# zrudnick/bramble

Measured on AMD Instinct MI355X. Metric: projected alignments/sec vs GENCODE-scale annotation, higher is better.
Workload: dtype u32

## Files before the change

bramble_amd/csrc/abi.cpp:

```cpp
#include <hip/hip_runtime.h>

#include <algorithm>
#include <atomic>
#include <cstdio>
#include <cstdlib>
#include <cstring>
#include <functional>
#include <string>
#include <thread>
#include <unordered_map>
#include <vector>

#include "ctx.h"
#include "primary_pick.h"

int check_device(int device) {
  int n = 0;
  hipError_t e = hipGetDeviceCount(&n);
  if (e != hipSuccess || n <= 0 || device >= n) return BR_ERR_NO_DEVICE;
  return BR_OK;
}

template <typename T>
static int upload(void **dst, const std::vector<T> &src, size_t &acc) {
// ... 66 lines not shown
  for (int pad = 0; pad < 4; pad++) ix->tx_ex.push_back(make_uint4(0xffffffffu, 0xffffffffu, 0, 0));
  auto for_each_par = [](size_t n, const std::function<void(size_t)> &fn) {
    unsigned hw = std::thread::hardware_concurrency();
    const size_t nt = std::min<size_t>(n, std::max(1u, std::min(hw ? hw : 1u, 16u)));
    if (nt <= 1) { for (size_t i = 0; i < n; i++) fn(i); return; }
    std::atomic<size_t> next{0};
    auto body = [&]() { for (;;) { const size_t i = next.fetch_add(1); if (i >= n) break; fn(i); } };
    std::vector<std::thread> th;
    for (size_t t = 1; t < nt; t++) th.emplace_back(body);
    body();
    for (auto &x : th) x.join();
  };
  ix->slab_off.assign(slabs.size() + 1, 0);
  {
    uint64_t tot = 0;
    for (size_t k = 0; k < slabs.size(); k++) { tot += slabs[k].size(); if (tot >= 0xfffffff0ull) { delete ix; return BR_ERR_CAPACITY; } ix->slab_off[k + 1] = (uint32_t)tot; }
    ix->s_start.resize((size_t)tot); ix->s_pmax.resize((size_t)tot); ix->s_tid.resize((size_t)tot); ix->s_row.resize((size_t)tot * 2);
  }
  for_each_par(slabs.size(), [&](size_t k) {
    auto &rows = slabs[k];
    std::stable_sort(rows.begin(), rows.end(), [](const Row &a, const Row &b) { return a.start < b.start; });
    uint32_t m = 0;
    size_t at = ix->slab_off[k];
    for (auto &r : rows) {
      m = std::max(m, r.end);
      ix->s_start[at] = r.start; ix->s_pmax[at] = m;
      ix->s_row[2 * at] = make_uint4(r.start, r.end, ix->tx_ex[ix->tx_first[r.tid] + r.gidx + 1].x , r.pos_start);
      const uint32_t n_ex = ix->tx_first[r.tid + 1] - ix->tx_first[r.tid] - 1;
      ix->s_row[2 * at + 1] = make_uint4(r.tid, r.gidx | (n_ex > 256u ? 0x80000000u : 0u), ix->tx_first[r.tid], ix->tx_ex[ix->tx_first[r.tid] + r.gidx + 1].y );
      ix->s_tid[at] = r.tid;
      at++;
    }
  });
  const uint32_t SHIFT = 10;
  std::vector<uint64_t> n_bins(ix->n_refs, 2);
  ix->bin_off.assign((size_t)ix->n_refs + 1, 0);
  {
    uint64_t tot = 0;
    for (uint32_t r = 0; r < ix->n_refs; r++) {
      uint64_t nb = 2;
      for (int sd = 0; sd < 2; sd++) {
        uint32_t sb = ix->slab_off[2 * r + sd], se = ix->slab_off[2 * r + sd + 1];
        if (se > sb) nb = std::max<uint64_t>(nb, ((uint64_t)std::max(ix->s_start[se - 1], ix->s_pmax[se - 1]) >> SHIFT) + 2);
      }
      n_bins[r] = nb;
      tot += nb + 1;
      if (tot >= 0xfffffff0ull) { delete ix; return BR_ERR_CAPACITY; }
      ix->bin_off[r + 1] = (uint32_t)tot;
    }
    ix->t_bin.resize((size_t)tot);
  }
  for_each_par(ix->n_refs, [&](size_t r) {
    const uint64_t nb = n_bins[r];
    const size_t first = ix->bin_off[r];
    for (int sd = 0; sd < 2; sd++) {
      uint32_t sb = ix->slab_off[2 * r + sd], se = ix->slab_off[2 * r + sd + 1];
      uint32_t rh = sb, rl = sb;
      for (uint64_t bk = 0; bk <= nb; bk++) {
        if (bk < nb) {
          uint64_t edge = bk << SHIFT;
          while (rh < se && (uint64_t)ix->s_start[rh] < edge) rh++;
          while (rl < se && (uint64_t)ix->s_pmax[rl] <= edge) rl++;
        } else rh = rl = se;
        uint4 &e = ix->t_bin[first + bk];
        if (sd == 0) { e.x = rl; e.y = rh; } else { e.z = rl; e.w = rh; }
      }
    }
// ... 329 lines not shown
```

bramble_amd/csrc/direct_kernels.inc:

```

#define WAVE_SYNC()                                                \
  do {                                                             \
    __builtin_amdgcn_fence(__ATOMIC_RELEASE, "workgroup");         \
    __builtin_amdgcn_wave_barrier();                               \
    __builtin_amdgcn_fence(__ATOMIC_ACQUIRE, "workgroup");         \
  } while (0)

__global__ void __launch_bounds__(256) k_name_seed(DirectArgs D) {
  const int64_t g = (int64_t)blockIdx.x * blockDim.x + threadIdx.x;
  if (g >= D.n_groups) return;
  const uint32_t a0 = D.group_off[g];
  const uint32_t no = D.name_off[a0];
  Mt64Lazy gen;
  gen.seed(hash_bytes(D.names + no, D.name_off[a0 + 1] - no));
  D.rnd0[g] = gen();
}
__device__ __forceinline__ uint32_t pick_from(uint64_t z0, const uint8_t *name, uint64_t len, uint32_t n) {
  uint64_t hi, lo;
  mul64wide(z0, (uint64_t)n, hi, lo);
  if (lo < (uint64_t)n) {
    const uint64_t thr = (0 - (uint64_t)n) % (uint64_t)n;
    if (lo < thr) return primary_pick(name, len, n);
  }
  return (uint32_t)hi;
// ... 416 lines not shown
    for (int k = 0; k < SCAN5_TOP_ITEMS; k++) { if (i0 + k < n_tiles) ts[i0 + k] = ex; ex += v[k]; }
    carry += tot;
  }
  if (threadIdx.x == 0) total_out[blockIdx.x] = carry;
}
__global__ void __launch_bounds__(256) k_scan5_apply(DirectArgs D, const uint64_t *tile_sums, int64_t n_tiles, const uint64_t *totals) {
  __shared__ uint64_t sh[4];
  const int64_t base = (int64_t)blockIdx.x * SCAN_TILE + (int64_t)threadIdx.x * SCAN_ITEMS;
  Scan5 v[SCAN_ITEMS];
  uint64_t sum[4] = {0, 0, 0, 0};
  scan5_load<false>(D, base, v);
#pragma unroll
  for (int k = 0; k < SCAN_ITEMS; k++)
#pragma unroll
    for (int c = 0; c < 4; c++) sum[c] += v[k].v[c];
  uint64_t ex[4];
#pragma unroll
  for (int c = 0; c < 4; c++) { uint64_t tot; ex[c] = block_excl_scan_256(sum[c], sh, tot) + tile_sums[(int64_t)c * n_tiles + blockIdx.x]; }
  const uint32_t n_simple = (uint32_t)totals[2];
  uint32_t o0[SCAN_ITEMS]; uint64_t o1[SCAN_ITEMS], o3[SCAN_ITEMS];
#pragma unroll
  for (int k = 0; k < SCAN_ITEMS; k++) {
    o0[k] = v[k].v[2] ? (uint32_t)ex[2] : n_simple + (uint32_t)(ex[0] - ex[2]);
    o1[k] = ex[1]; o3[k] = ex[3];
#pragma unroll
    for (int c = 0; c < 4; c++) ex[c] += v[k].v[c];
  }
  store8(D.cls_pos, base, D.n_aln, o0); store8(D.cig_base, base, D.n_aln, o1); store8(D.row_off, base, D.n_aln, o3);
  if (blockIdx.x == gridDim.x - 1 && threadIdx.x == 255) { D.cig_base[D.n_aln] = ex[1]; D.row_off[D.n_aln] = ex[3]; }
}

struct __attribute__((packed, aligned(4))) GD4 { uint32_t a, b, c, d; };
__global__ void __launch_bounds__(256) k_group_desc(DirectArgs D) {
  unsigned long long uniq = 0, dropped = 0;
  for (int64_t g = (int64_t)blockIdx.x * blockDim.x + threadIdx.x; g < D.n_groups; g += (int64_t)gridDim.x * blockDim.x) {
    const uint32_t a0 = D.group_off[g], a1 = D.group_off[g + 1];
    const uint32_t na = a1 - a0;
    uint32_t total = 0, units = 0, any = 0;
    uint32_t r4[4] = {0, 0, 0, 0}, f4[4] = {0, 0, 0, 0};
    int32_t mi4[4] = {-1, -1, -1, -1};
    const bool small = na <= 4u;
    if (small) {
      const GD4 rr = *(const GD4 *)(D.n_rows + a0), mm = *(const GD4 *)(D.n_matches + a0);
      typedef uint32_t u32u1 __attribute__((aligned(1)));
      const uint32_t ff = *(const u32u1 *)(D.pflag + a0);
#pragma unroll
      for (int k = 0; k < 4; k++) mi4[k] = (uint32_t)k < na ? D.mate_idx[a0 + (uint32_t)k] : -1;
      r4[0] = rr.a; r4[1] = rr.b; r4[2] = rr.c; r4[3] = rr.d;
      uint32_t m4[4] = {mm.a, mm.b, mm.c, mm.d};
#pragma unroll
      for (int k = 0; k < 4; k++) {
        f4[k] = (ff >> (8 * k)) & 0xffu;
        if ((uint32_t)k >= na) { r4[k] = 0; m4[k] = 0; f4[k] = 0; }
        total += r4[k]; units += (f4[k] & PF_PAIRED) ? r4[k] / 2 : r4[k]; any |= m4[k];
      }
    } else {
      for (uint32_t i = a0; i < a1; i++) { const uint32_t r = D.n_rows[i]; total += r; units += (D.pflag[i] & PF_PAIRED) ? r / 2 : r; any |= D.n_matches[i]; }
    }
    uniq += total == 1u ? 1 : 0;
    dropped += any ? 0 : 1;
    if (total == 0) continue;
    if (total > RR_HI) D.counters[3] = 1;
    const bool have_prim = D.names != nullptr;
    uint32_t idx = 0;
    if (have_prim && units > 1) {
      uint64_t hi, lo;
// ... 34 lines not shown
        const bool paired = (pf & PF_PAIRED) != 0;
        const uint32_t u = paired ? r / 2 : r;
        uint32_t prim = 0;
        if (have_prim && idx != 0xffffffffu) { if (idx < u) { prim = idx + 1u; idx = 0xffffffffu; } else idx -= u; }
        D.gd[i] = make_uint2(pf | (prim << 8), total);
        D.hi0[i] = run + 1u;
        if (paired) {
          const uint32_t m = (uint32_t)D.mate_idx[i];
          D.gd[m] = make_uint2((uint32_t)D.pflag[m] | (prim << 8), total);
          D.hi0[m] = run + 2u;
        }
        run += r;
      }
    }
  }
  __shared__ unsigned long long sh_c[4][2];
#pragma unroll
  for (int d = 32; d >= 1; d >>= 1) { uniq += __shfl_down(uniq, d, 64); dropped += __shfl_down(dropped, d, 64); }
  if ((threadIdx.x & 63) == 0) { sh_c[threadIdx.x >> 6][0] = uniq; sh_c[threadIdx.x >> 6][1] = dropped; }
  __syncthreads();
  if (threadIdx.x == 0) {
    const unsigned long long u = sh_c[0][0] + sh_c[1][0] + sh_c[2][0] + sh_c[3][0], dr = sh_c[0][1] + sh_c[1][1] + sh_c[2][1] + sh_c[3][1];
    uint64_t *slot = D.counters + GD_SLOT0 + (size_t)(blockIdx.x & (GD_SLOTS - 1)) * GD_SLOT_STRIDE;
    if (u) atomicAdd((unsigned long long *)&slot[0], u);
    if (dr) atomicAdd((unsigned long long *)&slot[1], dr);
  }
}

__global__ void __launch_bounds__(256) k_expand_rows(DirectArgs D) {
  __shared__ uint32_t sh_pre[4][64], sh_v[4][64];
  const int lane = threadIdx.x & 63, wv = threadIdx.x >> 6;
  const int64_t a = (int64_t)blockIdx.x * blockDim.x + threadIdx.x;
  if (D.m_aln_cap && D.tot[0] > D.m_aln_cap) return;
  uint32_t nk = 0, pos = 0, v = 0;
  bool fast = false;
  if (a < D.n_aln) nk = D.n_kept[a];
  if (nk) {
    fast = D.fast_flag[a] >> 31;
    pos = D.cls_pos[a];
    const uint32_t y = D.pflag[a];
    const bool is_mate = (y & PF_MATE) != 0;
    const uint32_t leader = is_mate ? (uint32_t)D.mate_idx[a] : (uint32_t)a;
    D.dpos[a] = make_uint2((uint32_t)D.row_off[leader] + (is_mate ? 1u : 0u), pos);
    v = (y & PF_BIG) ? 0xffffffffu : (uint32_t)a;
  }
  sh_v[wv][lane] = v;
#pragma unroll
  for (int c = 0; c < 2; c++) {
    const uint32_t mine = (nk && fast == (c == 0)) ? nk : 0u;
    const uint64_t have = __ballot(mine != 0u);
    if (!have) continue;
    uint32_t inc = mine;
#pragma unroll
    for (int d = 1; d < 64; d <<= 1) { const uint32_t up = __shfl_up(inc, d); if (lane >= d) inc += up; }
    const uint32_t total = __shfl(inc, 63), first = __shfl(pos, (int)__builtin_ctzll(have));
    __builtin_amdgcn_wave_barrier();
    sh_pre[wv][lane] = inc - mine;
    WAVE_SYNC();
    for (uint32_t e = lane; e < total; e += 64) {
      int l = 0;
#pragma unroll
      for (int st = 32; st; st >>= 1) if (sh_pre[wv][l + st] <= e) l += st;
      D.m_aln[first + e] = sh_v[wv][l];
    }
  }
}
// ... 149 lines not shown
```

bramble_amd/csrc/kernels.h:

```cpp
#pragma once
#include <hip/hip_runtime.h>
#include <stdint.h>

#include "device_types.h"
#include "ksw_types.h"

namespace br {

struct ProjectArgs {
  DevIndex ix;
  DevCfg cfg;
  int64_t n_aln;
  const int32_t *ref_id;
  const uint32_t *cigar_off;
  const uint32_t *cigar;
  const uint2 *seg;
  const AlnMeta *meta;
  const uint4 *head;
  const uint4 *head2;
  const uint32_t *fast_flag;
  const uint32_t *fast_pre;
  uint32_t *n_matches;
  uint4 *ranges;
  uint64_t *mask;
  uint32_t *big_list;
  uint32_t *n_big;
  uint32_t *walk_list;
  uint32_t *n_walk;
  uint32_t *m_aln;
  const uint32_t *match_off;
  const uint64_t *cig_base;
  uint32_t *m_tid, *m_aux;
  uint2 *m_p;
  uint2 *m_x;
  uint4 *m_b;
  uint64_t *m_cigoff;
  uint32_t *cig_arena;
  const uint64_t *tot;
  uint64_t lim_m, lim_c;
  uint64_t cover;
};
__device__ __forceinline__ bool tot_over(const uint64_t *tot, uint64_t lim_m, uint64_t lim_c) { return tot && (tot[0] > lim_m || tot[1] > lim_c); }

struct FaArgs {
  const int32_t *seq_src;
  const uint32_t *seq_off;
  const uint8_t *seqs;
  uint32_t *n_prob;
  uint32_t *seq_bytes;
  const uint32_t *prob_off;
  const uint64_t *seqarena_off;
  KswProb *probs;
  FaSrc *srcs;
  KswRes *results;
  uint8_t *seq_arena;
  uint32_t *clip_ops;
  uint32_t *ideal_cap;
  uint64_t *want_l, *want_r;
};

struct KswArgs {
  int64_t n_prob;
  const KswProb *probs;
  KswRes *results;
  const uint8_t *seq_arena;
  uint32_t *clip_ops;
  uint8_t *scratch;
  size_t scratch_per_wave, pmat_bytes, raw_words;
  int64_t n_waves;
  uint32_t tmax;
  uint64_t *stats;
  uint32_t *raw_out, *raw_n; int32_t *max_out; uint32_t raw_cap;
  const uint32_t *list; const uint32_t *n_list;
};

// ... 258 lines not shown
  int32_t *seq_src;
  uint32_t *seq_len;
  const uint32_t *seq_off;
  uint8_t *seqs;
  const int32_t *mate_ref_id, *mate_start;
};
struct SoaArgs {
  int64_t n;
  const uint64_t *cigar_off64, *name_off64, *seq_off64;
  uint32_t *cigar_off, *name_off, *seq_off;
  const uint8_t *names;
  const uint32_t *cigar;
  uint32_t *isnew;
  uint32_t *maxima;
};
void launch_soa_fields(hipStream_t st, const SoaArgs &S);
void launch_rec_fields(hipStream_t st, const ParseArgs &P);
void launch_group_off(hipStream_t st, const ParseArgs &P);
void launch_rec_copy(hipStream_t st, const ParseArgs &P);
void launch_mates(hipStream_t st, const ParseArgs &P);
void launch_seq_src(hipStream_t st, const ParseArgs &P);
void launch_seq_ascii(hipStream_t st, const ParseArgs &P);
void launch_bam_size(hipStream_t st, const BamArgs &B);
void launch_bam_encode(hipStream_t st, const BamArgs &B, int lanes);

struct SegExtra {
  const uint32_t *group_off; uint32_t *aln_group; int64_t n_groups;
  uint64_t *zero_a; int n_zero_a; uint64_t *zero_b; int n_zero_b;
};
void launch_segment(hipStream_t st, int64_t n_aln, const int32_t *ref_id, const int32_t *ref_start,
                    const uint16_t *flags, const int8_t *xs, const int8_t *ts, const uint32_t *cigar_off,
                    const uint32_t *cigar, const DevCfg &cfg, uint32_t n_refs, uint2 *seg, AlnMeta *meta,
                    uint4 *head, uint4 *head2, uint32_t *fast_flag, const SegExtra *extra = nullptr);
void launch_project(hipStream_t st, const ProjectArgs &A, bool emit, int group_lanes, int n_blocks, int part = 0);
void launch_project_fa(hipStream_t st, const ProjectArgs &A, const FaArgs &F, int mode, int n_blocks);
void launch_fa_fill(hipStream_t st, const ProjectArgs &A, const FaArgs &F, int64_t n_prob);
void launch_ksw(hipStream_t st, const KswArgs &K, int n_blocks);
void launch_ksw_bin(hipStream_t st, const KswFastArgs &A);
void launch_ksw_dp(hipStream_t st, const KswFastArgs &A, int bin);
void launch_ksw_trace(hipStream_t st, const KswFastArgs &A, int bin);
uint32_t ksw_dp_resident_groups(int bin, int n_cu);
size_t ksw_prob_bytes();
size_t ksw_res_bytes();
void launch_expand(hipStream_t st, const ProjectArgs &A);
void launch_emit_dense(hipStream_t st, const ProjectArgs &A, int64_t n_matches, int64_t n_simple, int part);
void launch_emit_dense_fa(hipStream_t st, const ProjectArgs &A, const FaArgs &F, int64_t n_matches);
int64_t scan_tiles_for(int64_t n);
void launch_scan(hipStream_t st, const ScanArgs &S, int mode, void *out, bool out64, uint64_t *total_out);
void launch_group_ids(hipStream_t st, int64_t n_groups, const uint32_t *group_off, uint32_t *aln_group);
bool launch_scan3(hipStream_t st, ScanArgs S, uint32_t *match_off, uint64_t *cig_base, uint32_t *fast_pre,
                  uint64_t *total_out3, const ProjectArgs *expand = nullptr);
void launch_pair(hipStream_t st, const PairArgs &P, bool emit);
void launch_primary(hipStream_t st, const PairArgs &P, const uint32_t *name_off, const uint8_t *names, bool has_scores);
void launch_rows(hipStream_t st, const PairArgs &P, bool aux);
void launch_rows_detail(hipStream_t st, const PairArgs &P);
void launch_pool_sizes(hipStream_t st, const PoolArgs &Q);
void launch_pool_copy(hipStream_t st, const PoolArgs &Q, bool long_cigars);
void launch_wide_fields(hipStream_t st, const WideArgs &W);
void launch_wide_cigars(hipStream_t st, const WideArgs &W, int64_t n_words);

}
```

bramble_amd/csrc/pipeline.cpp:

```cpp
#include <algorithm>
#include <cstring>
#include <vector>

#include "ctx.h"

int ensure_aux_stream(br_ctx *c) {
  if (c->ksw_stream) return BR_OK;
  HIPCHK(hipStreamCreateWithPriority(&c->ksw_stream, hipStreamNonBlocking, 0));
  for (auto &e : c->ksw_ev) HIPCHK(hipEventCreateWithFlags(&e, hipEventDisableTiming));
  for (auto &e : c->aux_ev) HIPCHK(hipEventCreateWithFlags(&e, hipEventDisableTiming));
  return BR_OK;
}

int run_ksw(br_ctx *c, hipStream_t st, const KswRun &R) {
  if (R.n_prob <= 0) return BR_OK;
  const uint64_t n_all = (uint64_t)R.n_prob;
  const uint64_t qmax = std::max<uint64_t>(R.qmax, 1), tmax = std::max<uint64_t>(R.tmax, 1);
  KswArgs K{};
  K.n_prob = R.n_prob; K.probs = R.probs; K.results = R.results; K.seq_arena = R.seq_arena; K.clip_ops = R.clip_ops;
  K.stats = R.stats;
  K.raw_out = R.raw_out; K.raw_n = R.raw_n; K.max_out = R.max_out; K.raw_cap = R.raw_cap;
  auto general = [&](uint64_t n_work, uint64_t q_hi, uint64_t t_hi, const uint32_t *list, const uint32_t *n_list) -> int {
    q_hi = std::max<uint64_t>(q_hi, 1); t_hi = std::max<uint64_t>(t_hi, 1);
    K.tmax = (uint32_t)t_hi;
// ... 75 lines not shown
        if (!A.n_bin[b]) continue;
        launch_ksw_dp(st, A, b);
        HIPCHK(hipEventRecord(c->ksw_ev[b], st));
        HIPCHK(hipStreamWaitEvent(c->ksw_stream, c->ksw_ev[b], 0));
        launch_ksw_trace(c->ksw_stream, A, b);
      }
      HIPCHK(hipEventRecord(c->ksw_ev[KSW_N_BINS], c->ksw_stream));
    }
    RC(general(n_left ? n_left : 64, std::max<uint64_t>(h_cnt[5], KSW_MAX_SPAN), std::max<uint64_t>(h_cnt[6], KSW_BIN_W(KSW_N_BINS - 1)), A.leftover, A.counters + KSW_N_BINS));
    if (n_groups_total) HIPCHK(hipStreamWaitEvent(st, c->ksw_ev[KSW_N_BINS], 0));
    HIPCHK(hipMemcpyAsync((uint32_t *)(c->h_totals + 24), A.counters + KSW_N_BINS, 4, hipMemcpyDeviceToHost, st));
  }
  return BR_OK;
}

static int ensure_count_tables(br_ctx *c, const br_device_batch *b) {
  const int64_t n = b->n_aln;
  RC(c->seg.ensure((size_t)(b->n_cigar_words + n) * sizeof(uint2)));
  RC(c->meta.ensure((size_t)n * sizeof(AlnMeta))); RC(c->head.ensure((size_t)n * sizeof(uint4))); RC(c->head2.ensure((size_t)n * sizeof(uint4)));
  RC(c->fast_flag.ensure((size_t)n * 4)); RC(c->ranges.ensure((size_t)n * sizeof(uint4))); RC(c->mask.ensure((size_t)n * 8));
  RC(c->cig_base.ensure((size_t)(n + 1) * 8)); RC(c->big_list.ensure((size_t)n * 4)); RC(c->totals.ensure(16 * 8));
  return BR_OK;
}

static ProjectArgs count_args(br_ctx *c, const DevCfg &dc, const br_device_batch *b) {
  ProjectArgs A{};
  A.ix = c->ix->dev; A.cfg = dc; A.n_aln = b->n_aln; A.ref_id = b->ref_id; A.cigar_off = b->cigar_off; A.cigar = b->cigar;
  A.seg = c->seg.as<uint2>(); A.meta = c->meta.as<AlnMeta>(); A.head = c->head.as<uint4>(); A.head2 = c->head2.as<uint4>();
  A.fast_flag = c->fast_flag.as<uint32_t>(); A.n_matches = c->n_matches.as<uint32_t>();
  A.ranges = c->ranges.as<uint4>(); A.mask = c->mask.as<uint64_t>(); A.big_list = c->big_list.as<uint32_t>();
  return A;
}

static int count_pass(br_ctx *c, hipStream_t st, const ProjectArgs &A, Prof &pf, bool split) {
  const int n_blocks = c->n_cu * c->blocks_per_cu;
  RC(pf.begin(BR_K_COUNT));
  launch_project(st, A, false, c->group_lanes, n_blocks, split ? 1 : 0);
  RC(pf.end());
  if (split) {
    RC(pf.begin(BR_K_COUNT_WALK));
    launch_project(st, A, false, c->group_lanes, n_blocks, 2);
    RC(pf.end());
  }
  return BR_OK;
}

static int emit_match_table(hipStream_t st, const ProjectArgs &A, Prof &pf, int64_t n_list, int64_t n_simple) {
  if (!A.cfg.filter_by_similarity) {
    RC(pf.begin(BR_K_EMIT_SIMPLE));
    launch_emit_dense(st, A, n_list, n_simple, 1);
    RC(pf.end());
    RC(pf.begin(BR_K_EMIT));
    launch_emit_dense(st, A, n_list, n_simple, 2);
    RC(pf.end());
  } else {
    RC(pf.begin(BR_K_EMIT));
    launch_emit_dense(st, A, n_list, -1, 0);
    RC(pf.end());
  }
  return BR_OK;
}

static void finish_call(br_ctx *c, const DevCfg &dc, const br_device_batch *b, br_device_rows *out, uint64_t n_matches,
                        uint64_t n_rows, uint64_t n_pool, bool aux_cols) {
  out->n_matches = (int64_t)n_matches; out->n_rows = (int64_t)n_rows; out->n_pool_words = (int64_t)n_pool;
  out->total_complete = n_rows; out->total_unique = c->h_totals[5]; out->dropped_reads = c->h_totals[6];
  out->pool = c->cig_arena.as<uint32_t>(); out->row_off = c->row_off.as<uint64_t>();
  c->counters[6] = n_matches;
  c->last_n_rows = (int64_t)n_rows; c->last_n_aln = b->n_aln; c->last_n_pool = (int64_t)n_pool;
  c->last_aux_cols = aux_cols; c->wide_valid = false; c->detail_valid = false; c->last_l_qseq = b->l_qseq; c->last_long_reads = dc.long_reads;
}

static int run_device_small(br_ctx *c, const DevCfg &dc, const br_device_batch *b, hipStream_t st, br_device_rows *out, Prof &pf,
                            bool keep_events, bool big) {
  const br_index *ix = c->ix;
  const int64_t n = b->n_aln, ng = b->n_groups;
// ... 683 lines not shown
```

bramble_amd/csrc/project_kernels.hip:

```cpp
#include <hip/hip_runtime.h>
#include <stdint.h>

#include <algorithm>

#include "device_types.h"
#include "kernels.h"
#include "primary_pick.h"

namespace br {

#define CIG_OP(c) ((c) & 0xfu)
#define CIG_LEN(c) ((c) >> 4)
#define CIG_GEN(l, o) (((l) << 4) | (o))

__global__ void __launch_bounds__(256) k_segment(int64_t n_aln, const int32_t *__restrict__ ref_id,
                                                 const int32_t *__restrict__ ref_start,
                                                 const uint16_t *__restrict__ flags,
                                                 const int8_t *__restrict__ xs, const int8_t *__restrict__ ts,
                                                 const uint32_t *__restrict__ cigar_off,
                                                 const uint32_t *__restrict__ cigar, DevCfg cfg,
                                                 uint32_t n_refs, uint2 *__restrict__ seg,
                                                 AlnMeta *__restrict__ meta, uint4 *__restrict__ head,
                                                 uint4 *__restrict__ head2, uint32_t *__restrict__ fast_flag, SegExtra X) {
  int64_t a = (int64_t)blockIdx.x * blockDim.x + threadIdx.x;
// ... 507 lines not shown
      uint4 pe = E[i_hit - 1];
      uint32_t len = pe.y - pe.x;
      sk.add(len, OP_D); acc.prev_op = OP_D; acc.ops += len; acc.cov += len; acc.ref_consumed += (int32_t)len;
      acc.junc_hits -= 2;
      k++;
    }
    if (R.ok && j == rd.n_seg - 1) h.right_ins = 0;
    build_match(acc, sk, h, status, q.x, q.y, ge.x, ge.y, k == 0, k == p1.n_gex - 1, L.ok, R.ok);
    k++;
    i_last = i_hit; e_last = ge; acc.last_pos = h.pos;
  }
  if (R.ok) { build_clip(acc, sk, R); k++; }
  if (acc.junc_hits < 0) acc.junc_hits = 0;
}

__device__ __forceinline__ bool similarity(const DevCfg &cfg, const Acc &acc, double &score) {
  score = 0.0;
  if (!cfg.filter_by_similarity) return true;
  double sim = (acc.ops > 0) ? (acc.cov / acc.ops) : 0.0;
  if (sim > cfg.thr) {
    double x = ((sim - cfg.thr) / (1.0 - cfg.thr));
    score = (x * x * (double)(acc.junc_hits + 1));
    return true;
  }
  return false;
}

#define SLAB_LDS 1025
#define WALK_LDS 2048
#define BIG_LDS 256
#define LDS_SLOT 25
#define LDS_IDEAL 10

template <int G, bool EMIT, bool SIMF, int MODE = 0>
__global__ void __launch_bounds__(256, EMIT ? 4 : 8) k_project(ProjectArgs A) {
  __shared__ uint32_t sh_slab[SLAB_LDS];
  __shared__ uint32_t sh_bin[EMIT ? 1 : SLAB_LDS];
  __shared__ uint32_t sh_cig[EMIT ? 256 * LDS_SLOT : 1];
  __shared__ uint32_t sh_wl[MODE == 1 ? WALK_LDS : 1];
  __shared__ uint32_t sh_wn, sh_wbase;
  __shared__ uint32_t sh_bl[EMIT ? 1 : BIG_LDS];
  __shared__ uint32_t sh_bn, sh_bbase;
  if (MODE == 1 || !EMIT) { if (threadIdx.x == 0) { sh_wn = 0; sh_bn = 0; } __syncthreads(); }
  const int gl = threadIdx.x & (G - 1);
  const int gbase = (threadIdx.x & 63) & ~(G - 1);
  const uint64_t gmask = (G == 64) ? ~0ull : ((1ull << G) - 1);
  const int64_t groups_total = (int64_t)gridDim.x * (blockDim.x / G);
  const int64_t gid = (int64_t)blockIdx.x * (blockDim.x / G) + threadIdx.x / G;
  const DevIndex &ix = A.ix;
  const DevCfg &cfg = A.cfg;
  const uint32_t n_slab_off = 2 * ix.n_refs + 1;
  const bool slab_in_lds = n_slab_off <= SLAB_LDS;
  if (slab_in_lds) {
    for (uint32_t i = threadIdx.x; i < n_slab_off; i += blockDim.x) {
      sh_slab[i] = ix.slab_off[i];
      if (!EMIT && i <= ix.n_refs) sh_bin[i] = ix.bin_off[i];
    }
    __syncthreads();
  }

  if (EMIT && tot_over(A.tot, A.lim_m, A.lim_c)) return;
  const int64_t n_work = EMIT ? (int64_t)*A.n_big : MODE == 2 ? (int64_t)*A.n_walk : A.n_aln;
  for (int64_t w = gid; w < n_work; w += groups_total) {
    const int64_t a = EMIT ? (int64_t)A.big_list[w] : MODE == 2 ? (int64_t)A.walk_list[w] : w;
    uint4 hd = A.head[a];
    uint4 hd2 = A.head2[a];
    uint32_t n_seg = hd.z;
    if (EMIT && n_seg == 0) continue;
    uint2 q0 = make_uint2(hd.x, hd.y);
    uint32_t smode = hd.w & 3u, rid = hd.w >> 2;
    int st0 = (n_seg == 1) ? ST_ONLY : ST_FIRST;
    uint32_t sb[2], se[2];
    if (slab_in_lds) { sb[0] = sh_slab[2 * rid]; se[0] = sh_slab[2 * rid + 1]; se[1] = sh_slab[2 * rid + 2]; }
    else { sb[0] = ix.slab_off[2 * rid]; se[0] = ix.slab_off[2 * rid + 1]; se[1] = ix.slab_off[2 * rid + 2]; }
    sb[1] = se[0];

    uint32_t lo[2] = {0, 0}, hi[2] = {0, 0};
    if (EMIT) {
      if (A.n_matches[a] == 0) continue;
      uint4 rg = A.ranges[a];
      lo[0] = rg.x; hi[0] = rg.y; lo[1] = rg.z; hi[1] = rg.w;
    } else {
      uint32_t tw[4];
      const uint32_t bo = slab_in_lds ? sh_bin[rid] : ix.bin_off[rid];
      const uint32_t nb = (slab_in_lds ? sh_bin[rid + 1] : ix.bin_off[rid + 1]) - bo - 1;
      uint32_t bh = q0.y >> ix.bin_shift, bl = q0.x >> ix.bin_shift;
      bh = bh < nb - 1 ? bh : nb - 1; bl = bl < nb - 1 ? bl : nb - 1;
      {
        const uint4 tl = ix.t_bin[bo + bl], th = ix.t_bin[bo + bh + 1];
        tw[0] = tl.x; tw[1] = th.y; tw[2] = tl.z; tw[3] = th.w;
      }
#pragma unroll
      for (int s = 0; s < 2; s++) {
        const bool use = ((smode >> s) & 1u) && sb[s] != se[s];
        hi[s] = use ? tw[2 * s + 1] : sb[s];
        lo[s] = use ? (tw[2 * s] < hi[s] ? tw[2 * s] : hi[s]) : sb[s];
      }
      if ((hi[0] - lo[0]) + (hi[1] - lo[1]) > 64u) {
        uint32_t ra[4], rb[4];
        const uint4 th0 = ix.t_bin[bo + bh], tl1 = ix.t_bin[bo + bl + 1];
#pragma unroll
        for (int s = 0; s < 2; s++) {
          ra[2 * s] = rb[2 * s] = ra[2 * s + 1] = rb[2 * s + 1] = sb[s];
          if (!((smode >> s) & 1u) || sb[s] == se[s]) continue;
          ra[2 * s] = s ? th0.w : th0.y; rb[2 * s] = hi[s];
          ra[2 * s + 1] = tw[2 * s]; rb[2 * s + 1] = s ? tl1.z : tl1.x;
        }
        uint32_t res[4] = {ra[0], ra[1], ra[2], ra[3]};
        for (uint32_t it = 0;; it += G) {
          bool any = false;
#pragma unroll
          for (int k = 0; k < 4; k++) any |= (ra[k] + it) < rb[k];
          if (!any) break;
#pragma unroll
          for (int k = 0; k < 4; k++) {
            uint32_t r = ra[k] + it + (uint32_t)gl;
            bool in = r < rb[k];
            uint32_t v = in ? ((k & 1) ? ix.s_pmax[r] : ix.s_start[r]) : 0u;
            bool t = in && ((k & 1) ? (v <= q0.x) : (v < q0.y));
            res[k] += (uint32_t)__popcll((__ballot(t) >> gbase) & gmask);
          }
        }
        hi[0] = res[0]; lo[0] = res[1] < res[0] ? res[1] : res[0];
        hi[1] = res[2]; lo[1] = res[3] < res[2] ? res[3] : res[2];
      }
      if (gl == 0) A.ranges[a] = make_uint4(lo[0], hi[0], lo[1], hi[1]);
    }
    uint32_t n0 = hi[0] - lo[0], n1 = hi[1] - lo[1];
    uint32_t n_items = n0 + n1;

    ReadCtx rd;
    rd.n_seg = n_seg; rd.seg = nullptr; rd.real = nullptr; rd.n_real = 0; rd.q12 = hd2;
    uint32_t moff = 0; uint64_t cbase = 0; uint32_t cap = 0, ideal_cap = 0;
    bool have_mask = false; uint64_t mask_in = 0;
    if (EMIT || n_seg > 3) {
      uint32_t c0 = A.cigar_off[a];
      rd.seg = A.seg + (size_t)c0 + (size_t)a;
      rd.real = A.cigar + c0;
      if (EMIT) rd.n_real = A.cigar_off[a + 1] - c0;
    }
    if (EMIT) {
      moff = A.match_off[a]; cbase = A.cig_base[a];
      ideal_cap = 4u * n_seg + 2u;
      cap = rd.n_real + 2u * ideal_cap;
      have_mask = n_items <= 64;
      mask_in = have_mask ? A.mask[a] : 0;
    }
    uint32_t total = 0;
    uint64_t mask_all = 0;
    bool defer = false;

    const int n_sweeps = (EMIT && !have_mask) ? 2 : 1;
    uint32_t aux_n = 0;
    for (int sweep = 0; sweep < n_sweeps; sweep++) {
      for (uint32_t base = 0; base < n_items; base += G) {
        uint32_t item = base + (uint32_t)gl;
        bool valid = item < n_items;
        bool alive = false;
        int s = 0; uint32_t row = 0, gs = 0, gend = 0, nxt = 0, nxe = 0;
        uint4 pay = make_uint4(0xffffffffu, 0, 0, 0);
        Hit h0; CandOut p1; const uint4 *E = nullptr; uint32_t i0 = 0;
        p1.alive = false; p1.fwpos = 0; p1.rcpos = 0; p1.n_seg = 0; p1.n_gex = 0;
        h0.pos = 0; h0.left_ins = h0.right_ins = h0.left_gap = h0.right_gap = 0;
        if (valid) {
          s = item < n0 ? 0 : 1;
          row = s == 0 ? lo[0] + item : lo[1] + (item - n0);
          const uint4 r_a = ix.s_row[2 * (size_t)row], r_b = ix.s_row[2 * (size_t)row + 1];
          gs = r_a.x; gend = r_a.y; nxt = r_a.z; nxe = r_b.w; pay = make_uint4(r_b.x, r_b.y, r_a.w, r_b.z);
          bool want = true;
          if (EMIT && have_mask) want = (mask_in >> item) & 1ull;
          if (want && gend > q0.x && gs < q0.y && classify(s == 1, st0, q0.x, q0.y, gs, gend, pay.z, cfg, h0)) {
            E = ix.tx_ex + pay.w; i0 = pay.y & 0x7fffffffu;
            bool superseded = false;
            if (nxt < q0.y) {
// ... 16 lines not shown
                  const bool c1 = nxt < qe1 && nxe > qs1 && classify(s == 1, ST_LAST, qs1, qe1, e1.x, e1.y, e1.z, cfg, hh);
                  alive2 = c1 && !c0;
                }
                p1.alive = alive2;
              }
              else if (MODE == 1 && !cfg.long_reads && !cfg.ignore_small_exons && !(pay.y >> 31)) {
                const uint32_t qs1 = hd2.x, qe1 = hd2.y;
                const int st1 = n_seg == 2 ? ST_LAST : ST_MIDDLE;
                Hit hh;
                if (gend < qe1 && !(qs1 == q0.x && qe1 == q0.y)) {
                  const bool c0 = gend > qs1 && classify(s == 1, st1, qs1, qe1, gs, gend, pay.z, cfg, hh);
                  const uint4 e1 = next_row(make_uint4(gs, gend, pay.z, 0), make_uint2(nxt, nxe), s == 1);
                  const bool c1 = nxt < qe1 && nxe > qs1 && classify(s == 1, st1, qs1, qe1, e1.x, e1.y, e1.z, cfg, hh);
                  if (c1 && !c0) defer = true;
                }
                p1.alive = false;
              }
              else if (MODE == 1) { defer = true; p1.alive = false; }
              else p1 = walk_pass1(ix, cfg, rd, E, s == 1, sb[s], se[s], i0, make_uint4(gs, gend, pay.z, 0), make_uint2(nxt, nxe), q0, h0);
              alive = p1.alive;
            }
          }
        }
        Acc acc; IdealSink sk; double score = 0.0;
        if (!EMIT || !have_mask) {
          if (SIMF && alive) {
            sk.init(nullptr);
            walk_pass2(ix, cfg, rd, E, s == 1, sb[s], se[s], i0, q0, make_uint4(gs, gend, pay.z, 0), make_uint2(nxt, nxe), h0, p1, acc, sk, no_clip(), no_clip());
            alive = similarity(cfg, acc, score);
          }
        }
        uint32_t rank = 0;
        bool do_emit = false;
        if (!EMIT) {
          uint64_t m = (__ballot(alive) >> gbase) & gmask;
          total += (uint32_t)__popcll(m);
          if (base < 64) mask_all |= (G == 64) ? m : (m << base);
        } else if (have_mask) {
          uint64_t mm = mask_in;
          while (mm) {
            int b = __ffsll((long long)mm) - 1; mm &= mm - 1;
            uint32_t t2;
            if ((uint32_t)b >= base && (uint32_t)b < base + G) t2 = __shfl(pay.x, b - (int)base, G);
            else {
              uint32_t r2 = (uint32_t)b < n0 ? lo[0] + (uint32_t)b : lo[1] + ((uint32_t)b - n0);
              t2 = ix.s_tid[r2];
            }
            rank += (t2 < pay.x) ? 1u : 0u;
          }
          do_emit = alive;
        } else {
          uint64_t m = (__ballot(alive) >> gbase) & gmask;
          if (sweep == 0) {
            if (alive) {
              uint32_t k = aux_n + (uint32_t)__popcll(m & ((1ull << gl) - 1ull));
              A.m_aux[moff + k] = pay.x;
            }
            aux_n += (uint32_t)__popcll(m);
          } else if (alive) {
            for (uint32_t k = 0; k < aux_n; k++) rank += (A.m_aux[moff + k] < pay.x) ? 1u : 0u;
            do_emit = true;
          }
        }
        if (EMIT && do_emit) {
          uint32_t *slot = A.cig_arena + cbase + (uint64_t)rank * cap;
          uint32_t *lds = &sh_cig[(EMIT ? threadIdx.x : 0) * LDS_SLOT];
          bool ideal_lds = ideal_cap <= LDS_IDEAL;
          uint32_t *ideal = ideal_lds ? lds : slot + rd.n_real + ideal_cap;
          sk.init(ideal);
          walk_pass2(ix, cfg, rd, E, s == 1, sb[s], se[s], i0, q0, make_uint4(gs, gend, pay.z, 0), make_uint2(nxt, nxe), h0, p1, acc, sk, no_clip(), no_clip());
          uint32_t n_ideal = sk.finish();
          similarity(cfg, acc, score);
          bool out_lds = ideal_lds && (rd.n_real + n_ideal <= LDS_SLOT - LDS_IDEAL);
          uint32_t *outp = out_lds ? lds + LDS_IDEAL : slot;
          RealCig rc; rc.fetch(rd.real, rd.n_real);
          uint32_t n_out = merge_cigars(rc, rd.n_real, ideal, n_ideal, outp);
          uint64_t cig_ref = cbase + (uint64_t)rank * cap;
          if (n_out <= 2) cig_ref = (uint64_t)(n_out > 0 ? outp[0] : 0u) | ((uint64_t)(n_out > 1 ? outp[1] : 0u) << 32);
          else if (out_lds) for (uint32_t k = 0; k < n_out; k++) slot[k] = outp[k];
          uint32_t mi = moff + rank;
          A.m_tid[mi] = pay.x;
          A.m_p[mi] = make_uint2((s == 0) ? p1.fwpos : p1.rcpos, n_out | ((uint32_t)s << 31));
          A.m_x[mi] = make_uint2((uint32_t)acc.junc_hits, (uint32_t)acc.ref_consumed);
          if (SIMF) {
            unsigned long long sb64 = (unsigned long long)__double_as_longlong(score);
            A.m_b[mi] = make_uint4((uint32_t)acc.clip_score, 0u, (uint32_t)sb64, (uint32_t)(sb64 >> 32));
          }
          A.m_cigoff[mi] = cig_ref;
        }
      }
      if (EMIT && !have_mask && sweep == 0) __threadfence_block();
    }
    if (MODE == 1 && ((__ballot(defer) >> gbase) & gmask) != 0) {
      if (gl == 0) {
        uint32_t k = atomicAdd(&sh_wn, 1u);
        if (k < WALK_LDS) sh_wl[MODE == 1 ? k : 0] = (uint32_t)a;
        else { uint32_t k2 = atomicAdd(A.n_walk, 1u); A.walk_list[k2] = (uint32_t)a; }
// ... 933 lines not shown
  constexpr int FG = FA_GROUP_LANES;
  int64_t need = (A.n_aln + (256 / FG) - 1) / (256 / FG);
  if (need < n_blocks) n_blocks = (int)need;
  if (n_blocks < 1) n_blocks = 1;
  dim3 g(n_blocks), b(256);
  switch (mode) {
    case 0: hipLaunchKernelGGL((k_project_fa<0, FG>), g, b, 0, st, A, F); break;
    case 1: hipLaunchKernelGGL((k_project_fa<1, FG>), g, b, 0, st, A, F); break;
    case 2: hipLaunchKernelGGL((k_project_fa<2, FG>), g, b, 0, st, A, F); break;
    default: hipLaunchKernelGGL((k_project_fa<3, FG>), g, b, 0, st, A, F); break;
  }
}

void launch_fa_fill(hipStream_t st, const ProjectArgs &A, const FaArgs &F, int64_t n_prob) {
  if (n_prob <= 0) return;
  int64_t blocks = std::min<int64_t>((n_prob + 15) / 16, 256 * 32);
  hipLaunchKernelGGL(k_fa_fill, dim3((unsigned)blocks), dim3(256), 0, st, A.ix.tx_ex, A.ix.seq_pool, F, n_prob);
}

static inline int grid_for(int64_t n, int per_block) { return (int)((n + per_block - 1) / per_block); }

void launch_segment(hipStream_t st, int64_t n_aln, const int32_t *ref_id, const int32_t *ref_start,
                    const uint16_t *flags, const int8_t *xs, const int8_t *ts, const uint32_t *cigar_off,
                    const uint32_t *cigar, const DevCfg &cfg, uint32_t n_refs, uint2 *seg, AlnMeta *meta,
                    uint4 *head, uint4 *head2, uint32_t *fast_flag, const SegExtra *extra) {
  if (n_aln <= 0) return;
  SegExtra X{};
  if (extra) X = *extra;
  hipLaunchKernelGGL(k_segment, dim3(grid_for(n_aln, 256)), dim3(256), 0, st, n_aln, ref_id, ref_start, flags,
                     xs, ts, cigar_off, cigar, cfg, n_refs, seg, meta, head, head2, fast_flag, X);
}

template <int G>
static void launch_project_g(hipStream_t st, const ProjectArgs &A, bool emit, int n_blocks, int part) {
  bool simf = A.cfg.filter_by_similarity != 0;
  if (emit) {
    if (simf) hipLaunchKernelGGL((k_project<G, true, true>), dim3(n_blocks), dim3(256), 0, st, A);
    else hipLaunchKernelGGL((k_project<G, true, false>), dim3(n_blocks), dim3(256), 0, st, A);
  } else {
    if (simf) hipLaunchKernelGGL((k_project<G, false, true>), dim3(n_blocks), dim3(256), 0, st, A);
    else if (A.walk_list) {
      if (part != 2) hipLaunchKernelGGL((k_project<G, false, false, 1>), dim3(n_blocks), dim3(256), 0, st, A);
      if (part != 1) hipLaunchKernelGGL((k_project<G, false, false, 2>), dim3(n_blocks), dim3(256), 0, st, A);
    } else hipLaunchKernelGGL((k_project<G, false, false>), dim3(n_blocks), dim3(256), 0, st, A);
  }
}

void launch_project(hipStream_t st, const ProjectArgs &A, bool emit, int group_lanes, int n_blocks, int part) {
  if (!emit && A.ix.n_rows == 0) {
    if (part == 2) return;
    (void)hipMemsetAsync(A.n_matches, 0, (size_t)A.n_aln * 4, st);
    (void)hipMemsetAsync(A.mask, 0, (size_t)A.n_aln * 8, st);
    (void)hipMemsetAsync(A.ranges, 0, (size_t)A.n_aln * sizeof(uint4), st);
    return;
  }
  if (A.n_aln <= 0) return;
  int64_t groups = A.n_aln;
  int per_block = 256 / group_lanes;
  int64_t need = (groups + per_block - 1) / per_block;
  if (need < n_blocks) n_blocks = (int)need;
  if (n_blocks < 1) n_blocks = 1;
  switch (group_lanes) {
    case 8: launch_project_g<8>(st, A, emit, n_blocks, part); break;
    case 16: launch_project_g<16>(st, A, emit, n_blocks, part); break;
    case 32: launch_project_g<32>(st, A, emit, n_blocks, part); break;
    default: launch_project_g<64>(st, A, emit, n_blocks, part); break;
  }
}

void launch_expand(hipStream_t st, const ProjectArgs &A) {
  if (A.n_aln <= 0) return;
  hipLaunchKernelGGL(k_expand, dim3(grid_for(A.n_aln, 256)), dim3(256), 0, st, A);
}

void launch_emit_dense(hipStream_t st, const ProjectArgs &A0, int64_t n_matches, int64_t n_simple, int part) {
  if (A0.n_aln <= 0 || n_matches <= 0) return;
  ProjectArgs A = A0;
  if (A.tot) A.cover = (uint64_t)(part == 1 ? n_simple : part == 2 ? n_matches - n_simple : n_matches);
  const FaArgs F{};
  if (A.cfg.filter_by_similarity) { hipLaunchKernelGGL((k_emit_dense<true, 0>), dim3(grid_for(n_matches, 256)), dim3(256), 0, st, A, (int64_t)0, n_matches, F); return; }
  if (part == 0 || n_simple < 0) { hipLaunchKernelGGL((k_emit_dense<false, 0>), dim3(grid_for(n_matches, 256)), dim3(256), 0, st, A, (int64_t)0, n_matches, F); return; }
  if (part == 1) { if (n_simple > 0) hipLaunchKernelGGL((k_emit_dense<false, 1>), dim3(grid_for(n_simple, 256)), dim3(256), 0, st, A, (int64_t)0, n_simple, F); }
  else if (n_matches > n_simple) hipLaunchKernelGGL((k_emit_dense<false, 2>), dim3(grid_for(n_matches - n_simple, 256)), dim3(256), 0, st, A, n_simple, n_matches, F);
}

void launch_emit_dense_fa(hipStream_t st, const ProjectArgs &A, const FaArgs &F, int64_t n_matches) {
  if (A.n_aln <= 0 || n_matches <= 0) return;
  hipLaunchKernelGGL((k_emit_dense<true, 0, true>), dim3(grid_for(n_matches, 256)), dim3(256), 0, st, A, (int64_t)0, n_matches, F);
}

int64_t scan_tiles_for(int64_t n) { return (n + SCAN_TILE - 1) / SCAN_TILE; }

void launch_scan(hipStream_t st, const ScanArgs &S, int mode, void *out, bool out64, uint64_t *total_out) {
  int64_t tiles = scan_tiles_for(S.n);
  if (tiles < 1) tiles = 1;
  dim3 g((unsigned)tiles), b(256);
  if (tiles <= SCAN_SMALL_TILES) {
    const dim3 one(1);
    if (mode == 1) hipLaunchKernelGGL((k_scan_small<1, uint64_t>), one, b, 0, st, S, (uint64_t *)out, total_out);
// ... 98 lines not shown
```

Measured before the change: 2.785 billion.

## Add slim CountArgs count kernels, halve bin width, early-exit group/expand kernels

```diff
diff --git a/bramble_amd/csrc/abi.cpp b/bramble_amd/csrc/abi.cpp
--- a/bramble_amd/csrc/abi.cpp
+++ b/bramble_amd/csrc/abi.cpp
@@ -122,7 +122,7 @@
       at++;
     }
   });
-  const uint32_t SHIFT = 10;
+  const uint32_t SHIFT = 9;
   std::vector<uint64_t> n_bins(ix->n_refs, 2);
   ix->bin_off.assign((size_t)ix->n_refs + 1, 0);
   {
diff --git a/bramble_amd/csrc/direct_kernels.inc b/bramble_amd/csrc/direct_kernels.inc
--- a/bramble_amd/csrc/direct_kernels.inc
+++ b/bramble_amd/csrc/direct_kernels.inc
@@ -472,6 +472,7 @@
 
 struct __attribute__((packed, aligned(4))) GD4 { uint32_t a, b, c, d; };
 __global__ void __launch_bounds__(256) k_group_desc(DirectArgs D) {
+  if (D.side_used[1]) return;
   unsigned long long uniq = 0, dropped = 0;
   for (int64_t g = (int64_t)blockIdx.x * blockDim.x + threadIdx.x; g < D.n_groups; g += (int64_t)gridDim.x * blockDim.x) {
     const uint32_t a0 = D.group_off[g], a1 = D.group_off[g + 1];
@@ -572,6 +573,7 @@
   const int lane = threadIdx.x & 63, wv = threadIdx.x >> 6;
   const int64_t a = (int64_t)blockIdx.x * blockDim.x + threadIdx.x;
   if (D.m_aln_cap && D.tot[0] > D.m_aln_cap) return;
+  if (D.side_used[1]) return;
   uint32_t nk = 0, pos = 0, v = 0;
   bool fast = false;
   if (a < D.n_aln) nk = D.n_kept[a];
diff --git a/bramble_amd/csrc/kernels.h b/bramble_amd/csrc/kernels.h
--- a/bramble_amd/csrc/kernels.h
+++ b/bramble_amd/csrc/kernels.h
@@ -41,6 +41,23 @@
   uint64_t cover;
 };
 __device__ __forceinline__ bool tot_over(const uint64_t *tot, uint64_t lim_m, uint64_t lim_c) { return tot && (tot[0] > lim_m || tot[1] > lim_c); }
+
+struct CountArgs {
+  const uint32_t *slab_off, *bin_off, *s_start, *s_pmax;
+  const uint4 *t_bin, *s_row, *tx_ex;
+  uint32_t n_refs, bin_shift;
+  uint32_t max_clip, max_junc_ins, max_junc_gap, max_error_exon;
+  int32_t ignore_small_exons, long_reads;
+  uint32_t n_aln;
+  const uint4 *head, *head2;
+  const uint32_t *cigar_off;
+  const uint2 *seg;
+  uint32_t *n_matches;
+  uint64_t *mask;
+  uint4 *ranges;
+  uint32_t *walk_list, *n_walk;
+  uint32_t *big_list, *n_big;
+};
 
 struct FaArgs {
   const int32_t *seq_src;
@@ -365,7 +382,8 @@
                     const uint16_t *flags, const int8_t *xs, const int8_t *ts, const uint32_t *cigar_off,
                     const uint32_t *cigar, const DevCfg &cfg, uint32_t n_refs, uint2 *seg, AlnMeta *meta,
                     uint4 *head, uint4 *head2, uint32_t *fast_flag, const SegExtra *extra = nullptr);
-void launch_project(hipStream_t st, const ProjectArgs &A, bool emit, int group_lanes, int n_blocks, int part = 0);
+void launch_project(hipStream_t st, const ProjectArgs &A, bool emit, int group_lanes, int n_blocks);
+void launch_count(hipStream_t st, const CountArgs &C, int group_lanes, int n_blocks, int part);
 void launch_project_fa(hipStream_t st, const ProjectArgs &A, const FaArgs &F, int mode, int n_blocks);
 void launch_fa_fill(hipStream_t st, const ProjectArgs &A, const FaArgs &F, int64_t n_prob);
 void launch_ksw(hipStream_t st, const KswArgs &K, int n_blocks);
diff --git a/bramble_amd/csrc/pipeline.cpp b/bramble_amd/csrc/pipeline.cpp
--- a/bramble_amd/csrc/pipeline.cpp
+++ b/bramble_amd/csrc/pipeline.cpp
@@ -131,16 +131,35 @@
   return A;
 }
 
+static CountArgs count_view(const ProjectArgs &A) {
+  CountArgs C{};
+  const DevIndex &ix = A.ix;
+  C.slab_off = ix.slab_off; C.bin_off = ix.bin_off; C.s_start = ix.s_start; C.s_pmax = ix.s_pmax;
+  C.t_bin = ix.t_bin; C.s_row = ix.s_row; C.tx_ex = ix.tx_ex; C.n_refs = ix.n_refs; C.bin_shift = ix.bin_shift;
+  C.max_clip = A.cfg.max_clip; C.max_junc_ins = A.cfg.max_junc_ins; C.max_junc_gap = A.cfg.max_junc_gap;
+  C.max_error_exon = A.cfg.max_error_exon; C.ignore_small_exons = A.cfg.ignore_small_exons; C.long_reads = A.cfg.long_reads;
+  C.n_aln = (uint32_t)A.n_aln;
+  C.head = A.head; C.head2 = A.head2; C.cigar_off = A.cigar_off; C.seg = A.seg;
+  C.n_matches = A.n_matches; C.mask = A.mask; C.ranges = A.ranges;
+  C.walk_list = A.walk_list; C.n_walk = A.n_walk; C.big_list = A.big_list; C.n_big = A.n_big;
+  return C;
+}
+
 static int count_pass(br_ctx *c, hipStream_t st, const ProjectArgs &A, Prof &pf, bool split) {
   const int n_blocks = c->n_cu * c->blocks_per_cu;
+  if (!split || A.ix.n_rows == 0) {
+    RC(pf.begin(BR_K_COUNT));
+    launch_project(st, A, false, c->group_lanes, n_blocks);
+    RC(pf.end());
+    return BR_OK;
+  }
+  const CountArgs C = count_view(A);
   RC(pf.begin(BR_K_COUNT));
-  launch_project(st, A, false, c->group_lanes, n_blocks, split ? 1 : 0);
-  RC(pf.end());
-  if (split) {
-    RC(pf.begin(BR_K_COUNT_WALK));
-    launch_project(st, A, false, c->group_lanes, n_blocks, 2);
-    RC(pf.end());
-  }
+  launch_count(st, C, c->group_lanes, n_blocks, 1);
+  RC(pf.end());
+  RC(pf.begin(BR_K_COUNT_WALK));
+  launch_count(st, C, c->group_lanes, n_blocks, 2);
+  RC(pf.end());
   return BR_OK;
 }
 
diff --git a/bramble_amd/csrc/project_kernels.hip b/bramble_amd/csrc/project_kernels.hip
--- a/bramble_amd/csrc/project_kernels.hip
+++ b/bramble_amd/csrc/project_kernels.hip
@@ -563,8 +563,25 @@
 #define LDS_SLOT 25
 #define LDS_IDEAL 10
 
-template <int G, bool EMIT, bool SIMF, int MODE = 0>
-__global__ void __launch_bounds__(256, EMIT ? 4 : 8) k_project(ProjectArgs A) {
+__device__ __forceinline__ const DevIndex &proj_index(const ProjectArgs &A) { return A.ix; }
+__device__ __forceinline__ DevIndex proj_index(const CountArgs &C) {
+  DevIndex ix{};
+  ix.n_refs = C.n_refs; ix.slab_off = C.slab_off; ix.s_start = C.s_start; ix.s_pmax = C.s_pmax; ix.s_row = C.s_row;
+  ix.tx_ex = C.tx_ex; ix.bin_shift = C.bin_shift; ix.bin_off = C.bin_off; ix.t_bin = C.t_bin;
+  return ix;
+}
+template <int PRE> __device__ __forceinline__ const DevCfg &proj_cfg(const ProjectArgs &A) { return A.cfg; }
+template <int PRE> __device__ __forceinline__ DevCfg proj_cfg(const CountArgs &C) {
+  DevCfg c{};
+  c.max_clip = C.max_clip; c.max_junc_ins = C.max_junc_ins; c.max_junc_gap = C.max_junc_gap;
+  c.max_error_exon = PRE ? 0u : C.max_error_exon;
+  c.ignore_small_exons = PRE ? 0 : C.ignore_small_exons;
+  c.long_reads = PRE ? 0 : C.long_reads;
+  return c;
+}
+
+template <int G, bool EMIT, bool SIMF, int MODE = 0, int PRE = 0, class Args = ProjectArgs>
+__global__ void __launch_bounds__(256, EMIT ? 4 : 8) k_project(Args A) {
   __shared__ uint32_t sh_slab[SLAB_LDS];
   __shared__ uint32_t sh_bin[EMIT ? 1 : SLAB_LDS];
   __shared__ uint32_t sh_cig[EMIT ? 256 * LDS_SLOT : 1];
@@ -576,10 +593,13 @@
   const int gl = threadIdx.x & (G - 1);
   const int gbase = (threadIdx.x & 63) & ~(G - 1);
   const uint64_t gmask = (G == 64) ? ~0ull : ((1ull << G) - 1);
-  const int64_t groups_total = (int64_t)gridDim.x * (blockDim.x / G);
-  const int64_t gid = (int64_t)blockIdx.x * (blockDim.x / G) + threadIdx.x / G;
-  const DevIndex &ix = A.ix;
-  const DevCfg &cfg = A.cfg;
+  constexpr bool CNT = std::is_same<Args, CountArgs>::value;
+  using Ix = typename std::conditional<CNT, uint32_t, int64_t>::type;
+  const uint32_t per_block = blockDim.x / G;
+  const Ix groups_total = (Ix)gridDim.x * per_block;
+  const Ix gid = (Ix)blockIdx.x * per_block + threadIdx.x / G;
+  const DevIndex &ix = proj_index(A);
+  const DevCfg &cfg = proj_cfg<PRE>(A);
   const uint32_t n_slab_off = 2 * ix.n_refs + 1;
   const bool slab_in_lds = n_slab_off <= SLAB_LDS;
   if (slab_in_lds) {
@@ -590,10 +610,10 @@
     __syncthreads();
   }
 
-  if (EMIT && tot_over(A.tot, A.lim_m, A.lim_c)) return;
-  const int64_t n_work = EMIT ? (int64_t)*A.n_big : MODE == 2 ? (int64_t)*A.n_walk : A.n_aln;
-  for (int64_t w = gid; w < n_work; w += groups_total) {
-    const int64_t a = EMIT ? (int64_t)A.big_list[w] : MODE == 2 ? (int64_t)A.walk_list[w] : w;
+  if constexpr (EMIT) { if (tot_over(A.tot, A.lim_m, A.lim_c)) return; }
+  const Ix n_work = EMIT ? (Ix)*A.n_big : MODE == 2 ? (Ix)*A.n_walk : (Ix)A.n_aln;
+  for (Ix w = gid; w < n_work; w += groups_total) {
+    const Ix a = EMIT ? (Ix)A.big_list[w] : MODE == 2 ? (Ix)A.walk_list[w] : w;
     uint4 hd = A.head[a];
     uint4 hd2 = A.head2[a];
     uint32_t n_seg = hd.z;
@@ -607,7 +627,7 @@
     sb[1] = se[0];
 
     uint32_t lo[2] = {0, 0}, hi[2] = {0, 0};
-    if (EMIT) {
+    if constexpr (EMIT) {
       if (A.n_matches[a] == 0) continue;
       uint4 rg = A.ranges[a];
       lo[0] = rg.x; hi[0] = rg.y; lo[1] = rg.z; hi[1] = rg.w;
@@ -667,10 +687,9 @@
     if (EMIT || n_seg > 3) {
       uint32_t c0 = A.cigar_off[a];
       rd.seg = A.seg + (size_t)c0 + (size_t)a;
-      rd.real = A.cigar + c0;
-      if (EMIT) rd.n_real = A.cigar_off[a + 1] - c0;
-    }
-    if (EMIT) {
+      if constexpr (EMIT) { rd.real = A.cigar + c0; rd.n_real = A.cigar_off[a + 1] - c0; }
+    }
+    if constexpr (EMIT) {
       moff = A.match_off[a]; cbase = A.cig_base[a];
       ideal_cap = 4u * n_seg + 2u;
       cap = rd.n_real + 2u * ideal_cap;
@@ -753,7 +772,7 @@
         }
         uint32_t rank = 0;
         bool do_emit = false;
-        if (!EMIT) {
+        if constexpr (!EMIT) {
           uint64_t m = (__ballot(alive) >> gbase) & gmask;
           total += (uint32_t)__popcll(m);
           if (base < 64) mask_all |= (G == 64) ? m : (m << base);
@@ -783,7 +802,8 @@
             do_emit = true;
           }
         }
-        if (EMIT && do_emit) {
+        if constexpr (EMIT) {
+          if (!do_emit) continue;
           uint32_t *slot = A.cig_arena + cbase + (uint64_t)rank * cap;
           uint32_t *lds = &sh_cig[(EMIT ? threadIdx.x : 0) * LDS_SLOT];
           bool ideal_lds = ideal_cap <= LDS_IDEAL;
@@ -1783,39 +1803,62 @@
 }
 
 template <int G>
-static void launch_project_g(hipStream_t st, const ProjectArgs &A, bool emit, int n_blocks, int part) {
+static void launch_project_g(hipStream_t st, const ProjectArgs &A, bool emit, int n_blocks) {
   bool simf = A.cfg.filter_by_similarity != 0;
   if (emit) {
     if (simf) hipLaunchKernelGGL((k_project<G, true, true>), dim3(n_blocks), dim3(256), 0, st, A);
     else hipLaunchKernelGGL((k_project<G, true, false>), dim3(n_blocks), dim3(256), 0, st, A);
   } else {
     if (simf) hipLaunchKernelGGL((k_project<G, false, true>), dim3(n_blocks), dim3(256), 0, st, A);
-    else if (A.walk_list) {
-      if (part != 2) hipLaunchKernelGGL((k_project<G, false, false, 1>), dim3(n_blocks), dim3(256), 0, st, A);
-      if (part != 1) hipLaunchKernelGGL((k_project<G, false, false, 2>), dim3(n_blocks), dim3(256), 0, st, A);
-    } else hipLaunchKernelGGL((k_project<G, false, false>), dim3(n_blocks), dim3(256), 0, st, A);
-  }
-}
-
-void launch_project(hipStream_t st, const ProjectArgs &A, bool emit, int group_lanes, int n_blocks, int part) {
+    else hipLaunchKernelGGL((k_project<G, false, false>), dim3(n_blocks), dim3(256), 0, st, A);
+  }
+}
+
+static int project_blocks(int64_t n_aln, int group_lanes, int n_blocks) {
+  const int per_block = 256 / group_lanes;
+  const int64_t need = (n_aln + per_block - 1) / per_block;
+  if (need < n_blocks) n_blocks = (int)need;
+  return n_blocks < 1 ? 1 : n_blocks;
+}
+
+void launch_project(hipStream_t st, const ProjectArgs &A, bool emit, int group_lanes, int n_blocks) {
   if (!emit && A.ix.n_rows == 0) {
-    if (part == 2) return;
     (void)hipMemsetAsync(A.n_matches, 0, (size_t)A.n_aln * 4, st);
     (void)hipMemsetAsync(A.mask, 0, (size_t)A.n_aln * 8, st);
     (void)hipMemsetAsync(A.ranges, 0, (size_t)A.n_aln * sizeof(uint4), st);
     return;
   }
   if (A.n_aln <= 0) return;
-  int64_t groups = A.n_aln;
-  int per_block = 256 / group_lanes;
-  int64_t need = (groups + per_block - 1) / per_block;
-  if (need < n_blocks) n_blocks = (int)need;
-  if (n_blocks < 1) n_blocks = 1;
+  n_blocks = project_blocks(A.n_aln, group_lanes, n_blocks);
   switch (group_lanes) {
-    case 8: launch_project_g<8>(st, A, emit, n_blocks, part); break;
-    case 16: launch_project_g<16>(st, A, emit, n_blocks, part); break;
-    case 32: launch_project_g<32>(st, A, emit, n_blocks, part); break;
-    default: launch_project_g<64>(st, A, emit, n_blocks, part); break;
+    case 8: launch_project_g<8>(st, A, emit, n_blocks); break;
+    case 16: launch_project_g<16>(st, A, emit, n_blocks); break;
+    case 32: launch_project_g<32>(st, A, emit, n_blocks); break;
+    default: launch_project_g<64>(st, A, emit, n_blocks); break;
+  }
+}
+
+template <int G>
+static void launch_count_g(hipStream_t st, const CountArgs &C, int n_blocks, int part) {
+  const bool pre = !C.long_reads && !C.ignore_small_exons;
+  const dim3 g(n_blocks), b(256);
+  if (part == 1) {
+    if (pre) hipLaunchKernelGGL((k_project<G, false, false, 1, 1, CountArgs>), g, b, 0, st, C);
+    else hipLaunchKernelGGL((k_project<G, false, false, 1, 0, CountArgs>), g, b, 0, st, C);
+  } else {
+    if (pre) hipLaunchKernelGGL((k_project<G, false, false, 2, 1, CountArgs>), g, b, 0, st, C);
+    else hipLaunchKernelGGL((k_project<G, false, false, 2, 0, CountArgs>), g, b, 0, st, C);
+  }
+}
+
+void launch_count(hipStream_t st, const CountArgs &C, int group_lanes, int n_blocks, int part) {
+  if (C.n_aln == 0) return;
+  n_blocks = project_blocks(C.n_aln, group_lanes, n_blocks);
+  switch (group_lanes) {
+    case 8: launch_count_g<8>(st, C, n_blocks, part); break;
+    case 16: launch_count_g<16>(st, C, n_blocks, part); break;
+    case 32: launch_count_g<32>(st, C, n_blocks, part); break;
+    default: launch_count_g<64>(st, C, n_blocks, part); break;
   }
 }
 
```

Result: faster. 2.853 billion, median of 6 (+2.4%).
